# kmaninis/OSVOS-PyTorch

Measured on NVIDIA H100. Metric: frames/sec at 480x854 fwd-only, batch 1 per GPU (OSVOS.forward -> 5 logit maps), higher is better.
Workload: dtype bf16x3 (split-bf16 operands, fp32 accumulate)

## Files before the change

### include/osvos_b200.h

```cpp
#ifndef OSVOS_B200_H_
#define OSVOS_B200_H_

#include <stddef.h>
#include <stdint.h>

#ifdef __cplusplus
extern "C" {
#endif

#define OSVOS_B200_VERSION 100

#if defined(__GNUC__)
#define OSVOS_API __attribute__((visibility("default")))
#else
#define OSVOS_API
#endif

enum {
  OSVOS_OK = 0,
  OSVOS_ERR_INVALID_ARGUMENT = 1,
  OSVOS_ERR_CUDA = 2,
  OSVOS_ERR_UNSUPPORTED = 3
};

// ... 11 lines not shown
OSVOS_API int osvos_version(void);
OSVOS_API const char* osvos_last_error(void);
OSVOS_API int osvos_set_pdl(int mode);

OSVOS_API size_t osvos_packed_weight_bytes(int rows, int cols_padded);
OSVOS_API int osvos_pack_conv3x3_weights(const float* w_oihw, void* packed, int cout, int cin, int transpose_flip,
                               int col_pad, osvos_stream_t stream);

OSVOS_API int osvos_nchw_to_act(const float* x_nchw, void* act_hi, void* act_lo, int n, int c, int h, int w,
                      osvos_stream_t stream);
OSVOS_API int osvos_act_to_nchw(const void* act_hi, const void* act_lo, float* y_nchw, int n, int c, int h, int w,
                      osvos_stream_t stream);

OSVOS_API int osvos_conv_first_fwd(const float* x_nchw, const float* w_oihw, const float* bias, void* y_hi, void* y_lo,
                         int n, int h, int w, int flags, osvos_stream_t stream);

typedef struct {
  const void* x_hi;
  const void* x_lo;
  const void* w_packed;
  const float* bias;
  void* y_hi;
  void* y_lo;
  float* y_f32;
  const void* mask_hi;
  const float* proj_w;
  const float* proj_b;
  float* pq;
  void* pool_hi;
  void* pool_lo;
  float* colsum;
  int n, h, w, cin, cout;
  int flags;
} osvos_conv3x3_args;
OSVOS_API int osvos_conv3x3(const osvos_conv3x3_args* args , osvos_stream_t stream);

OSVOS_API int osvos_fold_side_weights(const float* side_w , const float* side_b ,
                                      const float* proj_w , const float* proj_b , void* packed,
                                      float* bias2 , int cin, osvos_stream_t stream);
OSVOS_API int osvos_side_folded_multi(const osvos_conv3x3_args* args , int count, osvos_stream_t stream);

typedef struct {
  const float* side_w;
  const float* side_b;
  const float* proj_w;
  const float* proj_b;
  void* packed;
  float* bias2;
  float* folded_f32;
  int cin;
} osvos_fold_item;
OSVOS_API int osvos_fold_side_weights_multi(const osvos_fold_item* items , int count, osvos_stream_t stream);
OSVOS_API int osvos_conv3x3_simt(const osvos_conv3x3_args* args , osvos_stream_t stream);

typedef struct {
  const float* x;
  const float* w1;
  const float* b1;
  const void* w2_packed;
  const float* b2;
  void* y_hi;
  void* y_lo;
  void* pool_hi;
  void* pool_lo;
  int n, h, w;
} osvos_stage1_args;
OSVOS_API int osvos_stage1_fused(const osvos_stage1_args* args , osvos_stream_t stream);

// ... 293 lines not shown
```

### osvos_pytorch_b200/_native.py

```python
import ctypes
import os
from ctypes import (POINTER, Structure, c_char_p, c_double, c_float, c_int, c_int32, c_size_t, c_uint32, c_uint64,
                    c_void_p)

_HERE = os.path.dirname(os.path.abspath(__file__))
LIB_PATH = os.path.join(_HERE, "lib", "libosvos_b200.so")

FLAG_RELU = 1
FLAG_FAST = 2
FLAG_RELU_MASK = 4
FLAG_ACCUMULATE = 8
FLAG_DEFER_FINISH = 16
FLAG_DETERMINISTIC = 32
WGRAD_FINISH_MAX = 24


class NativeLibraryError(RuntimeError):
    pass


class Conv3x3Args(Structure):
    _fields_ = [("x_hi", c_void_p), ("x_lo", c_void_p), ("w_packed", c_void_p), ("bias", c_void_p),
                ("y_hi", c_void_p), ("y_lo", c_void_p), ("y_f32", c_void_p), ("mask_hi", c_void_p),
                ("proj_w", c_void_p), ("proj_b", c_void_p), ("pq", c_void_p),
                ("pool_hi", c_void_p), ("pool_lo", c_void_p), ("colsum", c_void_p),
                ("n", c_int), ("h", c_int), ("w", c_int), ("cin", c_int), ("cout", c_int), ("flags", c_int)]


class Stage1Args(Structure):
    _fields_ = [("x", c_void_p), ("w1", c_void_p), ("b1", c_void_p), ("w2_packed", c_void_p), ("b2", c_void_p),
                ("y_hi", c_void_p), ("y_lo", c_void_p), ("pool_hi", c_void_p), ("pool_lo", c_void_p),
                ("n", c_int), ("h", c_int), ("w", c_int)]


class TailFwdArgs(Structure):
    _fields_ = [("pq", c_void_p * 4), ("fuse_bias", c_void_p), ("out", c_void_p * 5), ("label", c_void_p),
                ("sums", c_void_p), ("losses", c_void_p), ("loss_weights", c_float * 5), ("divisor", c_float),
                ("n", c_int), ("h", c_int), ("w", c_int), ("flags", c_int)]


TAIL_SUMS = 15


class TailLossBwdArgs(Structure):
    _fields_ = [("logits", c_void_p * 5), ("label", c_void_p), ("sums", c_void_p), ("upstream", c_void_p),
                ("loss_weights", c_float * 5), ("divisor", c_float), ("dpq", c_void_p * 4), ("fuse_bias_grad", c_void_p),
                ("n", c_int), ("h", c_int), ("w", c_int), ("flags", c_int)]


class WgradArgs(Structure):
    _fields_ = [("x_hi", c_void_p), ("x_lo", c_void_p), ("dz_hi", c_void_p), ("dz_lo", c_void_p), ("dw", c_void_p),
                ("workspace", c_void_p), ("n", c_int), ("h", c_int), ("w", c_int), ("cin", c_int), ("cout", c_int),
                ("dz_channels", c_int), ("flags", c_int)]


class WgradFinishItem(Structure):
    _fields_ = [("workspace", c_void_p), ("dw", c_void_p), ("cout", c_int), ("cin", c_int), ("dz_channels", c_int),
                ("accumulate", c_int), ("scale", c_float)]

# ... 43 lines not shown
                ("losses", c_void_p), ("loss_weights", c_float * 5), ("divisor", c_float), ("n", c_int), ("h", c_int),
                ("w", c_int), ("flags", c_int)]


class TailGeneralBwdArgs(Structure):
    _fields_ = [("feat", c_void_p * 4), ("pq", c_void_p * 4), ("score_w", c_void_p * 4), ("vtab", c_void_p),
                ("atab", c_void_p), ("src", c_void_p * 5), ("label", c_void_p), ("sums", c_void_p),
                ("upstream", c_void_p), ("loss_weights", c_float * 5), ("divisor", c_float), ("df_hi", c_void_p * 4),
                ("df_lo", c_void_p * 4), ("red", c_void_p * 4), ("fuse_bias_grad", c_void_p), ("workspace", c_void_p),
                ("n", c_int), ("h", c_int), ("w", c_int), ("flags", c_int)]


class UpsamplingGradsArgs(Structure):
    _fields_ = [("red", c_void_p * 4), ("upscale_w", c_void_p * 4), ("fuse_w", c_void_p), ("d_upscale_w", c_void_p * 4),
                ("d_upscale1_w", c_void_p * 4), ("d_fuse_w", c_void_p), ("d_score_w", c_void_p * 4),
                ("d_score_b", c_void_p * 4), ("d_side_b", c_void_p * 4), ("accumulate", c_int)]


UPSAMPLING_TAPS = 1360
U8_PROB, U8_BYTESCALE, U8_MASK = 0, 1, 2
RESIZE_BILINEAR, RESIZE_NEAREST = 0, 1
SGD_MAX_SEGMENTS = 64

SIGNATURES = {
    "osvos_version": (c_int, []),
    "osvos_last_error": (c_char_p, []),
    "osvos_packed_weight_bytes": (c_size_t, [c_int, c_int]),
    "osvos_pack_conv3x3_weights": (c_int, [c_void_p, c_void_p, c_int, c_int, c_int, c_int, c_void_p]),
    "osvos_nchw_to_act": (c_int, [c_void_p, c_void_p, c_void_p, c_int, c_int, c_int, c_int, c_void_p]),
    "osvos_act_to_nchw": (c_int, [c_void_p, c_void_p, c_void_p, c_int, c_int, c_int, c_int, c_void_p]),
    "osvos_conv_first_fwd": (c_int, [c_void_p, c_void_p, c_void_p, c_void_p, c_void_p, c_int, c_int, c_int, c_int,
                                     c_void_p]),
    "osvos_conv3x3": (c_int, [POINTER(Conv3x3Args), c_void_p]),
    "osvos_stage1_fused": (c_int, [POINTER(Stage1Args), c_void_p]),
    "osvos_set_pdl": (c_int, [c_int]),
    "osvos_fold_side_weights": (c_int, [c_void_p, c_void_p, c_void_p, c_void_p, c_void_p, c_void_p, c_int, c_void_p]),
    "osvos_side_folded_multi": (c_int, [POINTER(Conv3x3Args), c_int, c_void_p]),
    "osvos_fold_side_weights_multi": (c_int, [POINTER(FoldItem), c_int, c_void_p]),
    "osvos_conv3x3_simt": (c_int, [POINTER(Conv3x3Args), c_void_p]),
    "osvos_maxpool2x2_fwd": (c_int, [c_void_p, c_void_p, c_void_p, c_void_p, c_int, c_int, c_int, c_int, c_void_p]),
    "osvos_tail_fwd": (c_int, [POINTER(TailFwdArgs), c_void_p]),
    "osvos_cbce_fwd": (c_int, [c_void_p, c_void_p, c_size_t, c_double, c_void_p, c_void_p, c_void_p]),
    "osvos_cbce_bwd": (c_int, [c_void_p, c_void_p, c_void_p, c_void_p, c_double, c_size_t, c_void_p, c_void_p]),
    "osvos_wgrad_workspace_bytes": (c_size_t, [c_int, c_int]),
    "osvos_conv3x3_wgrad": (c_int, [POINTER(WgradArgs), c_void_p]),
    "osvos_wgrad_finish": (c_int, [POINTER(WgradFinishItem), c_int, c_void_p]),
    "osvos_tail_bwd": (c_int, [POINTER(TailBwdArgs), c_void_p]),
    "osvos_tail_loss_bwd": (c_int, [POINTER(TailLossBwdArgs), c_void_p]),
    "osvos_sum_f32": (c_int, [c_void_p, c_size_t, c_void_p, c_void_p, c_void_p]),
    "osvos_unpool_add_mask": (c_int, [c_void_p, c_void_p, c_void_p, c_void_p, c_void_p, c_void_p, c_void_p, c_void_p,
                                      c_int, c_int, c_int, c_int, c_void_p]),
    "osvos_side_folded_wgrad_floats": (c_size_t, [c_int]),
    "osvos_side_folded_wgrad": (c_int, [c_void_p, c_void_p, c_void_p, c_void_p, c_int, c_int, c_int, c_int, c_void_p]),
    "osvos_side_folded_wgrad_multi": (c_int, [POINTER(SideWgradItem), c_int, c_void_p]),
    "osvos_side_grads_finish": (c_int, [POINTER(SideGradsItem), c_int, c_void_p]),
    "osvos_unpool_side_mask": (c_int, [c_void_p, c_void_p, c_void_p, c_void_p, c_void_p, c_void_p, c_void_p, c_void_p,
                                       c_void_p, c_int, c_int, c_int, c_int, c_void_p]),
    "osvos_channel_sum": (c_int, [c_void_p, c_void_p, c_void_p, c_size_t, c_int, c_void_p]),
    "osvos_conv_first_bwd_workspace_bytes": (c_size_t, []),
    "osvos_conv_first_bwd": (c_int, [c_void_p, c_void_p, c_void_p, c_void_p, c_void_p, c_void_p, c_void_p, c_int, c_int, c_int,
                                     c_void_p]),
    "osvos_side_project": (c_int, [c_void_p, c_void_p, c_void_p, c_void_p, c_int, c_int, c_int, c_void_p]),
    "osvos_logits_to_u8": (c_int, [c_void_p, c_void_p, c_void_p, c_int, c_size_t, c_int, c_void_p]),
    "osvos_sgd_work_items": (c_uint32, [c_uint64, c_int, c_int]),
    "osvos_sgd_step": (c_int, [c_void_p, c_int, c_uint32, c_int, c_void_p]),
    "osvos_affine_warp": (c_int, [c_void_p, c_void_p, POINTER(c_double), POINTER(c_int), c_int, c_int, c_int, c_int,
# ... 83 lines not shown
```

### osvos_pytorch_b200/csrc/conv3x3_halo.cu

```cuda
#include "conv_common.cuh"

namespace osvos {

constexpr int kHaloRows = kTileH + 2;
constexpr int kPitch = kTileW + 2;

template <int BLOCK_N, int PLANES, bool SPLIT>
struct HaloCfg {
  static constexpr int kABoxBytes = kHaloRows * kPitch * 128;
  static constexpr int kAPlaneBytes = (kABoxBytes + 1023) / 1024 * 1024;
  static constexpr int kAStageBytes = PLANES * kAPlaneBytes;
  static constexpr int kAStages = 2;
  static constexpr int kBPlaneBytes = BLOCK_N * 128;
  static constexpr int kBStageBytes = PLANES * kBPlaneBytes;
  static constexpr int kBudget = 225 * 1024 - kAStages * kAStageBytes;
  static constexpr int kBStagesRaw = kBudget / kBStageBytes;
  static constexpr int kBStages = kBStagesRaw > 9 ? 9 : kBStagesRaw;
  static constexpr bool kSplitAcc = SPLIT;
  static_assert(!SPLIT || (PLANES == 2 && BLOCK_N <= 128), "split accumulators need two planes and 2 * BLOCK_N <= 256");
  static constexpr int kAccCols = kSplitAcc ? 2 * BLOCK_N : BLOCK_N;
  static constexpr int kAcc = kAccCols / 2;
  static constexpr int kSmemBytes = kAStages * kAStageBytes + kBStages * kBStageBytes + 1024 + 512;
  static_assert(kBStages >= 2, "weight ring too shallow");
  static_assert(kSmemBytes <= 227 * 1024, "more than the per-CTA shared memory of sm_90");
  static_assert(kSmemBytes + 4096 < (1 << 18), "descriptor start-address field would overflow");
  static_assert(kBStageBytes % 1024 == 0, "B stage must keep 1024-byte alignment");
};

template <int BLOCK_N, int PLANES, bool SPLIT, bool LEAN, bool PINGPONG, bool DET = false>
__global__ void __launch_bounds__(kConvThreads, 1)
conv3x3_halo_kernel(const __grid_constant__ CUtensorMap map_x_hi, const __grid_constant__ CUtensorMap map_x_lo,
                    const __grid_constant__ CUtensorMap map_w_hi, const __grid_constant__ CUtensorMap map_w_lo,
                    const ConvParams p) {
  using Cfg = HaloCfg<BLOCK_N, PLANES, SPLIT>;
  constexpr int SA = Cfg::kAStages, SB = Cfg::kBStages;
  constexpr int kHalves = PINGPONG ? 2 : 1;
  static_assert(!PINGPONG || kHalves * Cfg::kAcc <= 128, "a ping-pong warpgroup holds the whole tile's accumulator");

  extern __shared__ uint8_t smem_raw[];
  uint8_t* smem = reinterpret_cast<uint8_t*>((reinterpret_cast<uintptr_t>(smem_raw) + 1023) & ~uintptr_t(1023));
  uint8_t* smem_a = smem;
  uint8_t* smem_b = smem + SA * Cfg::kAStageBytes;
  uint64_t* bars = reinterpret_cast<uint64_t*>(smem_b + SB * Cfg::kBStageBytes);
  uint64_t* a_full = bars;
  uint64_t* a_empty = bars + SA;
  uint64_t* b_full = bars + 2 * SA;
  uint64_t* b_empty = bars + 2 * SA + SB;

  const int warp = threadIdx.x >> 5;
  const int lane = threadIdx.x & 31;

  if (warp == 0 && lane == 0) {
    tma_prefetch_desc(&map_x_hi);
    tma_prefetch_desc(&map_w_hi);
    if (PLANES == 2) {
      tma_prefetch_desc(&map_x_lo);
      tma_prefetch_desc(&map_w_lo);
    }
    constexpr uint32_t kReaders = PINGPONG ? 1 : 2;
    for (int i = 0; i < SA; ++i) {
      mbar_init(&a_full[i], 1);
      mbar_init(&a_empty[i], kReaders);
    }
    for (int i = 0; i < SB; ++i) {
      mbar_init(&b_full[i], 1);
      mbar_init(&b_empty[i], kReaders);
    }
    fence_barrier_init();
  }
  __syncthreads();
  pdl_wait();
  pdl_launch_dependents();

  if (warp < 4) {
    if (PINGPONG) setmaxnreg_dec<40>();
    if (warp != 0) return;
    if (elect_one()) {
      int a_stage = 0, b_stage = 0;
      uint32_t a_phase = 0, b_phase = 0;
      const bool skip_a = (p.ablate & 2) != 0, skip_b = (p.ablate & 1) != 0;
      auto issue_a = [&](int x0, int y0, int img, int kc) {
        mbar_wait(&a_empty[a_stage], a_phase ^ 1);
        if (skip_a) {
          mbar_arrive(&a_full[a_stage]);
        } else {
          uint8_t* st = smem_a + a_stage * Cfg::kAStageBytes;
          mbar_arrive_expect_tx(&a_full[a_stage], PLANES * Cfg::kABoxBytes);
          tma_load_4d(&map_x_hi, &a_full[a_stage], st, kc * kBlockK, x0, y0, img);
          if (PLANES == 2) tma_load_4d(&map_x_lo, &a_full[a_stage], st + Cfg::kAPlaneBytes, kc * kBlockK, x0, y0, img);
        }
        if (++a_stage == SA) {
          a_stage = 0;
          a_phase ^= 1;
        }
      };
      int nb = 0, tx = 0, ty = 0, img = 0;
      const int w_first = static_cast<int>(blockIdx.x), w_stride = static_cast<int>(gridDim.x);
      if (w_first < p.total_tiles) {
        decode_tile(p, w_first, nb, tx, ty, img);
        issue_a(tx * kTileW - 1, ty * kTileH - 1, img, 0);
      }
      for (int tile = w_first; tile < p.total_tiles; tile += w_stride) {
        const bool has_next = tile + w_stride < p.total_tiles;
        int nnb = 0, ntx = 0, nty = 0, nimg = 0;
        if (has_next) decode_tile(p, tile + w_stride, nnb, ntx, nty, nimg);
        const int n0 = nb * BLOCK_N;
        for (int kc = 0; kc < p.k_chunks; ++kc) {
          const int c0 = kc * kBlockK;
#pragma unroll
          for (int tap = 0; tap < 9; ++tap) {
            if (tap == 3) {
              if (kc + 1 < p.k_chunks) issue_a(tx * kTileW - 1, ty * kTileH - 1, img, kc + 1);
              else if (has_next) issue_a(ntx * kTileW - 1, nty * kTileH - 1, nimg, 0);
            }
            mbar_wait(&b_empty[b_stage], b_phase ^ 1);
            if (skip_b) {
              mbar_arrive(&b_full[b_stage]);
            } else {
              uint8_t* st = smem_b + b_stage * Cfg::kBStageBytes;
              mbar_arrive_expect_tx(&b_full[b_stage], Cfg::kBStageBytes);
              tma_load_3d(&map_w_hi, &b_full[b_stage], st, c0, n0, tap);
              if (PLANES == 2) tma_load_3d(&map_w_lo, &b_full[b_stage], st + Cfg::kBPlaneBytes, c0, n0, tap);
            }
            if (++b_stage == SB) {
              b_stage = 0;
              b_phase ^= 1;
            }
          }
        }
        nb = nnb, tx = ntx, ty = nty, img = nimg;
      }
    }
    __syncwarp();
  } else {
    if (PINGPONG) setmaxnreg_inc<232>();
    const int wg = (warp - 4) >> 2, wl = warp & 3;
    const bool leader = (threadIdx.x & 127) == 0;
    constexpr uint64_t kDescA = desc_template(16, kPitch * 128, kDescSW128);
    constexpr uint64_t kDescB = desc_template(16, 1024, kDescSW128);
    constexpr uint32_t kLoPlaneA = Cfg::kAPlaneBytes >> 4, kLoPlaneB = Cfg::kBPlaneBytes >> 4;
    constexpr uint32_t kHalfA = (8 * kPitch * 128) >> 4;
    const uint32_t smem_a_u32 = smem_u32(smem_a) + (PINGPONG ? 0 : wg * 8 * kPitch * 128), smem_b_u32 = smem_u32(smem_b);
    const bool skip_mma = (p.ablate & 4) != 0;
    float acc[kHalves][Cfg::kAcc];
    StageRelease pending;
    constexpr int kOwners = PINGPONG ? 2 : 1;
    for (int k = PINGPONG ? wg : 0;; k += kOwners) {
      const int tile = static_cast<int>(blockIdx.x) + k * static_cast<int>(gridDim.x);
      if (tile >= p.total_tiles) break;
      const bool has_next = tile + static_cast<int>(gridDim.x) < p.total_tiles;
      const int a_seq = k * p.k_chunks, b_seq = 9 * a_seq;
      int a_stage = a_seq % SA, b_stage = b_seq % SB;
      uint32_t a_phase = (a_seq / SA) & 1, b_phase = (b_seq / SB) & 1;
      if (PINGPONG && k > 0) named_bar_sync(1 + wg, 256);
#pragma unroll
      for (int h = 0; h < kHalves; ++h)
#pragma unroll
        for (int i = 0; i < Cfg::kAcc; ++i) acc[h][i] = 0.f;
      for (int kc = 0; kc < p.k_chunks; ++kc) {
        mbar_wait(&a_full[a_stage], a_phase);
        const uint64_t da0 = kDescA | static_cast<uint64_t>((smem_a_u32 + a_stage * Cfg::kAStageBytes) >> 4);
#pragma unroll
        for (int tap = 0; tap < 9; ++tap) {
          const uint32_t tap_off = static_cast<uint32_t>(((tap / 3) * kPitch + (tap % 3)) * (128 >> 4));
          mbar_wait(&b_full[b_stage], b_phase);
          if (PINGPONG && tap == 8 && kc == p.k_chunks - 1 && has_next) named_bar_arrive(1 + (wg ^ 1), 256);
          const uint64_t db_hi = kDescB | static_cast<uint64_t>((smem_b_u32 + b_stage * Cfg::kBStageBytes) >> 4);
          wgmma_fence();
#pragma unroll
          for (int h = 0; h < kHalves; ++h) {
            const uint64_t da_hi = da0 + h * kHalfA + tap_off;
            const uint64_t da_lo = da_hi + kLoPlaneA;
            if (skip_mma) continue;
#pragma unroll
            for (int ks = 0; ks < kBlockK / 16; ++ks) {
              if constexpr (Cfg::kSplitAcc) {
                wgmma_bf16<2 * BLOCK_N>(acc[h], da_hi + 2 * ks, db_hi + 2 * ks, 1);
                wgmma_bf16<BLOCK_N>(acc[h], da_lo + 2 * ks, db_hi + 2 * ks, 1);
              } else if constexpr (PLANES == 2) {
                wgmma_bf16<BLOCK_N>(acc[h], da_lo + 2 * ks, db_hi + 2 * ks, 1);
                wgmma_bf16<BLOCK_N>(acc[h], da_hi + 2 * ks, db_hi + kLoPlaneB + 2 * ks, 1);
                wgmma_bf16<BLOCK_N>(acc[h], da_hi + 2 * ks, db_hi + 2 * ks, 1);
              } else {
                wgmma_bf16<BLOCK_N>(acc[h], da_hi + 2 * ks, db_hi + 2 * ks, 1);
              }
            }
          }
          wgmma_commit();
          wgmma_wait<1>();
          pending.release(leader);
          pending.bar_b = &b_empty[b_stage];
          if (tap == 8) pending.bar_a = &a_empty[a_stage];
          if (++b_stage == SB) {
            b_stage = 0;
            b_phase ^= 1;
          }
        }
        if (++a_stage == SA) {
          a_stage = 0;
          a_phase ^= 1;
        }
      }
      wgmma_wait<0>();
#pragma unroll
      for (int h = 0; h < kHalves; ++h) wgmma_fence_operands(acc[h]);
      pending.release(leader);
#pragma unroll
      for (int h = 0; h < kHalves; ++h)
        conv_epilogue<BLOCK_N, Cfg::kSplitAcc, LEAN, DET>(p, acc[h], tile, PINGPONG ? h : wg, wl, lane);
    }
  }
}

template <int BLOCK_N, int PLANES, bool LEAN = false, bool DET = false>
static int launch_halo(const osvos_conv3x3_args* a, cudaStream_t stream) {
  constexpr bool kSplit = PLANES == 2 && BLOCK_N <= 128;
  using Cfg = HaloCfg<BLOCK_N, PLANES, kSplit>;
  ConvParams p;
  fill_conv_params(p, a, BLOCK_N);
  const int sms = device_sm_count();
  CUtensorMap mx_hi, mx_lo, mw_hi, mw_lo;
  {
    const uint64_t dims[4] = {(uint64_t)a->cin, (uint64_t)a->w, (uint64_t)a->h, (uint64_t)a->n};
    const uint64_t strides[3] = {(uint64_t)a->cin * 2, (uint64_t)a->w * a->cin * 2,
                                 (uint64_t)a->h * a->w * a->cin * 2};
    const uint32_t box[4] = {kBlockK, kPitch, kHaloRows, 1};
    int rc = encode_tensor_map(&mx_hi, CU_TENSOR_MAP_DATA_TYPE_BFLOAT16, 2, 4, a->x_hi, dims, strides, box,
                               CU_TENSOR_MAP_SWIZZLE_128B);
    if (rc) return rc;
    rc = encode_tensor_map(&mx_lo, CU_TENSOR_MAP_DATA_TYPE_BFLOAT16, 2, 4, PLANES == 2 ? a->x_lo : a->x_hi, dims,
                           strides, box, CU_TENSOR_MAP_SWIZZLE_128B);
    if (rc) return rc;
  }
  int rc = encode_weight_maps(&mw_hi, &mw_lo, a, BLOCK_N);
  if (rc) return rc;
  const int grid = p.total_tiles < sms ? p.total_tiles : sms;
  constexpr bool kCanPingPong = BLOCK_N == 64 || BLOCK_N == 128;
  const bool pingpong = kCanPingPong && p.total_tiles > 2 * sms;
  auto kern = pingpong ? conv3x3_halo_kernel<BLOCK_N, PLANES, kSplit && BLOCK_N == 64, LEAN, kCanPingPong, DET>
                       : conv3x3_halo_kernel<BLOCK_N, PLANES, kSplit, LEAN, false, DET>;
  static uint64_t attr_done[2] = {0, 0};
  OSVOS_CHECK_CUDA(ensure_dynamic_smem(kern, Cfg::kSmemBytes, &attr_done[pingpong]));
  OSVOS_CHECK_CUDA(launch_pdl(kern, dim3(grid), dim3(kConvThreads), Cfg::kSmemBytes, stream, mx_hi, mx_lo,
                              mw_hi, mw_lo, p));
  return OSVOS_OK;
}

template <bool DET>
static int conv3x3_halo_dispatch(const osvos_conv3x3_args* a, cudaStream_t stream) {
  const bool fast = (a->flags & OSVOS_FLAG_FAST) != 0;
  const bool lean = !fast && !(a->flags & OSVOS_FLAG_RELU_MASK) && a->colsum == nullptr && a->y_f32 == nullptr;
  const int m_tiles = ((a->w + kTileW - 1) / kTileW) * ((a->h + kTileH - 1) / kTileH) * a->n;
  const int sms = device_sm_count();
  const long tiles128 = static_cast<long>(m_tiles) * (a->cout / 128);
  const long waves128 = (tiles128 + sms - 1) / sms;
  const long waves256 = (static_cast<long>(m_tiles) * (a->cout / 256) + sms - 1) / sms;
  if (a->cout == 64 || (waves128 == 1 && tiles128 * 5 <= static_cast<long>(sms) * 3)) {
    if (lean) return launch_halo<64, 2, true>(a, stream);
    return fast ? launch_halo<64, 1, false, DET>(a, stream) : launch_halo<64, 2, false, DET>(a, stream);
  }
  const bool prefer256 = fast ? waves256 * 1100 < waves128 * 700 : waves256 * 2200 < waves128 * 1000;
  if (a->cout % 256 == 0 && prefer256)
    return fast ? launch_halo<256, 1, false, DET>(a, stream) : launch_halo<256, 2, false, DET>(a, stream);
  if (fast) return launch_halo<128, 1, false, DET>(a, stream);
  if (lean) return launch_halo<128, 2, true>(a, stream);
  return launch_halo<128, 2, false, DET>(a, stream);
}

static int check_conv_args(const osvos_conv3x3_args* a) {
  OSVOS_CHECK_ARG(a != nullptr);
  OSVOS_CHECK_ARG(a->n > 0 && a->h > 0 && a->w > 0);
  OSVOS_CHECK_ARG(a->cin >= 64 && a->cin % 64 == 0);
  OSVOS_CHECK_ARG(a->cout == 2 || a->cout == 16 || a->cout == 64 || (a->cout > 0 && a->cout % 128 == 0));
  OSVOS_CHECK_ARG(a->cout != 2 || (a->pq != nullptr && a->y_hi == nullptr && a->y_f32 == nullptr && a->pool_hi == nullptr &&
                                   a->colsum == nullptr && !(a->flags & (OSVOS_FLAG_RELU | OSVOS_FLAG_RELU_MASK))));
  OSVOS_CHECK_ARG(a->cout != 16 || (a->y_hi == nullptr && a->y_lo == nullptr && !(a->flags & OSVOS_FLAG_RELU_MASK)));
  OSVOS_CHECK_ARG(a->x_hi != nullptr && a->w_packed != nullptr);
  OSVOS_CHECK_ARG((a->flags & OSVOS_FLAG_FAST) || a->x_lo != nullptr);
  OSVOS_CHECK_ARG(a->y_hi != nullptr || a->y_f32 != nullptr || a->pq != nullptr || a->pool_hi != nullptr);
  OSVOS_CHECK_ARG(!(a->flags & OSVOS_FLAG_RELU_MASK) || a->mask_hi != nullptr);
  OSVOS_CHECK_ARG(a->pq == nullptr || a->cout == 2 || (a->cout == 16 && a->proj_w != nullptr));
  OSVOS_CHECK_ARG((a->pool_hi == nullptr && a->colsum == nullptr) || a->cout >= 64);
  OSVOS_CHECK_ARG((reinterpret_cast<uintptr_t>(a->x_hi) & 15) == 0);
  OSVOS_CHECK_ARG((reinterpret_cast<uintptr_t>(a->w_packed) & 15) == 0);
  OSVOS_CHECK_ARG((reinterpret_cast<uintptr_t>(a->bias) & 15) == 0);
  OSVOS_CHECK_ARG(!(a->flags & OSVOS_FLAG_DETERMINISTIC) || (reinterpret_cast<uintptr_t>(a->colsum) & 7) == 0);
  if (a->cout >= 64) {
    const uintptr_t bf16_planes = reinterpret_cast<uintptr_t>(a->y_hi) | reinterpret_cast<uintptr_t>(a->y_lo) |
                                  reinterpret_cast<uintptr_t>(a->pool_hi) | reinterpret_cast<uintptr_t>(a->pool_lo) |
                                  reinterpret_cast<uintptr_t>(a->mask_hi);
    OSVOS_CHECK_ARG((bf16_planes & 3) == 0);
    OSVOS_CHECK_ARG((reinterpret_cast<uintptr_t>(a->y_f32) & 7) == 0);
  }
// ... 2 lines not shown

}

using namespace osvos;

extern "C" int osvos_side_folded_multi(const osvos_conv3x3_args* args, int count, osvos_stream_t stream_) {
  OSVOS_CHECK_ARG(args != nullptr && count > 0 && count <= 4);
  const osvos_conv3x3_args* order[4];
  for (int k = 0; k < count; ++k) {
    int rc = check_conv_args(&args[k]);
    if (rc) return rc;
    OSVOS_CHECK_ARG(args[k].cout == 2);
    OSVOS_CHECK_ARG((args[k].flags & OSVOS_FLAG_FAST) == (args[0].flags & OSVOS_FLAG_FAST));
    order[k] = &args[k];
  }
  for (int i = 1; i < count; ++i)
    for (int j = i; j > 0 && order[j]->cin > order[j - 1]->cin; --j) {
      const osvos_conv3x3_args* t = order[j];
      order[j] = order[j - 1];
      order[j - 1] = t;
    }
  return side_conv_multi_dispatch(order, count, static_cast<cudaStream_t>(stream_));
}

extern "C" int osvos_conv3x3(const osvos_conv3x3_args* a, osvos_stream_t stream_) {
  int rc = check_conv_args(a);
  if (rc) return rc;
  cudaStream_t stream = static_cast<cudaStream_t>(stream_);
  if (a->cout == 2 || a->cout == 16) return side_conv_dispatch(a, stream);
  if ((a->flags & OSVOS_FLAG_DETERMINISTIC) && a->colsum != nullptr) return conv3x3_halo_dispatch<true>(a, stream);
  return conv3x3_halo_dispatch<false>(a, stream);
}

extern "C" size_t osvos_conv3x3_colsum_rows(int n, int h, int w) {
  if (n <= 0 || h <= 0 || w <= 0) return 0;
  return static_cast<size_t>(n) * ((h + kTileH - 1) / kTileH) * ((w + kTileW - 1) / kTileW) * 8;
}
```

### osvos_pytorch_b200/csrc/conv_common.cuh

```cuda
#pragma once
#include <stdlib.h>

#include "common.cuh"
#include "ptx.cuh"

namespace osvos {

constexpr int kTileW = 8;
constexpr int kTileH = 16;
constexpr int kBlockM = 128;
constexpr int kBlockK = 64;
constexpr int kConvThreads = 384;
constexpr int kABytes = kBlockM * kBlockK * 2;

struct ConvParams {
  const float* bias;
  __nv_bfloat16* y_hi;
  __nv_bfloat16* y_lo;
  float* y_f32;
  const __nv_bfloat16* mask_hi;
  __nv_bfloat16* pool_hi;
  __nv_bfloat16* pool_lo;
  float* colsum;
  int n, h, w, cin, cout;
  int tiles_x, tiles_y, n_blocks, total_tiles, k_chunks;
  int flags;
  int ablate;
};

__device__ __forceinline__ void decode_tile(const ConvParams& p, int tile, int& nb, int& tx, int& ty, int& img) {
  nb = tile % p.n_blocks;
  int m = tile / p.n_blocks;
  tx = m % p.tiles_x;
  m /= p.tiles_x;
  ty = m % p.tiles_y;
  img = m / p.tiles_y;
}

__device__ __forceinline__ uint32_t sw128_offset(int row, int chunk) { return row * 128 + ((chunk ^ (row & 7)) << 4); }

__device__ __forceinline__ void split_pack2(float a, float b, uint32_t& hi, uint32_t& lo) {
  asm("cvt.rn.bf16x2.f32 %0, %1, %2;" : "=r"(hi) : "f"(b), "f"(a));
  const float ra = a - __uint_as_float(hi << 16);
  const float rb = b - __uint_as_float(hi & 0xFFFF0000u);
  asm("cvt.rn.bf16x2.f32 %0, %1, %2;" : "=r"(lo) : "f"(rb), "f"(ra));
}

template <int BLOCK_N, bool SPLIT_ACC, bool LEAN = false, bool DET = false>
__device__ __forceinline__ void conv_epilogue(const ConvParams& p, const float* acc, int tile, int wg, int wl, int lane) {
  if (p.ablate & 16) return;
  int nb, tx, ty, img;
  decode_tile(p, tile, nb, tx, ty, img);
  const int lx = lane >> 2;
  const int x = tx * kTileW + lx;
  const int y0 = ty * kTileH + wg * 8 + wl * 2;
  const bool va = (y0 < p.h) && (x < p.w), vb = (y0 + 1 < p.h) && (x < p.w);
  const bool relu = (p.flags & OSVOS_FLAG_RELU) != 0;
  const bool masked = !LEAN && (p.flags & OSVOS_FLAG_RELU_MASK) != 0;
  const bool store_ok = !(p.ablate & 8);
  const size_t pix[2] = {(static_cast<size_t>(img) * p.h + y0) * p.w + x, (static_cast<size_t>(img) * p.h + y0 + 1) * p.w + x};
// ... 109 lines not shown
        st_shared_u32(act_row + h * 8 * 128 + ((j ^ lx) << 4) + col, plane ? lo : hi);
      }
    }
    fence_proxy_async_smem();
    named_bar_sync(bar_id, 128);
    if (leader && store_ok) {
      tma_store_4d(plane ? &maps.y_lo : &maps.y_hi, box, nb * 64, tx * kTileW, ty * kTileH + half * 8, img);
      bulk_commit_group();
    }
  }
}


static inline void fill_conv_params(ConvParams& p, const osvos_conv3x3_args* a, int block_n) {
  p.bias = a->bias;
  p.y_hi = static_cast<__nv_bfloat16*>(a->y_hi);
  p.y_lo = static_cast<__nv_bfloat16*>(a->y_lo);
  p.y_f32 = a->y_f32;
  p.mask_hi = static_cast<const __nv_bfloat16*>(a->mask_hi);
  p.pool_hi = static_cast<__nv_bfloat16*>(a->pool_hi);
  p.pool_lo = static_cast<__nv_bfloat16*>(a->pool_lo);
  p.colsum = a->colsum;
  p.n = a->n;
  p.h = a->h;
  p.w = a->w;
  p.cin = a->cin;
  p.cout = a->cout;
  p.tiles_x = (a->w + kTileW - 1) / kTileW;
  p.tiles_y = (a->h + kTileH - 1) / kTileH;
  p.n_blocks = a->cout / block_n;
  p.total_tiles = p.tiles_x * p.tiles_y * a->n * p.n_blocks;
  p.k_chunks = a->cin / kBlockK;
  p.flags = a->flags;
  {
    static int ablate = -1;
    if (ablate < 0) {
      const char* e = getenv("OSVOS_ABLATE");
      ablate = e ? atoi(e) : 0;
    }
    p.ablate = ablate;
  }
}

static inline int encode_weight_maps(CUtensorMap* hi, CUtensorMap* lo, const osvos_conv3x3_args* a, int block_n) {
  const size_t plane = static_cast<size_t>(9) * a->cout * a->cin;
  const uint64_t dims[3] = {(uint64_t)a->cin, (uint64_t)a->cout, 9};
  const uint64_t strides[2] = {(uint64_t)a->cin * 2, (uint64_t)a->cout * a->cin * 2};
  const uint32_t box[3] = {kBlockK, (uint32_t)block_n, 1};
  const __nv_bfloat16* wp = static_cast<const __nv_bfloat16*>(a->w_packed);
  int rc = encode_tensor_map(hi, CU_TENSOR_MAP_DATA_TYPE_BFLOAT16, 2, 3, wp, dims, strides, box,
                             CU_TENSOR_MAP_SWIZZLE_128B);
  if (rc) return rc;
  return encode_tensor_map(lo, CU_TENSOR_MAP_DATA_TYPE_BFLOAT16, 2, 3, wp + plane, dims, strides, box,
                           CU_TENSOR_MAP_SWIZZLE_128B);
}

static inline bool outputs_tma_aligned(const osvos_conv3x3_args* a) {
  return ((reinterpret_cast<uintptr_t>(a->y_hi) | reinterpret_cast<uintptr_t>(a->y_lo)) & 15) == 0;
}

static inline int encode_output_maps(OutMaps* m, const osvos_conv3x3_args* a) {
  memset(m, 0, sizeof(*m));
  const uint64_t c = a->cout;
  const uint64_t dims[4] = {c, (uint64_t)a->w, (uint64_t)a->h, (uint64_t)a->n};
  const uint64_t strides[3] = {c * 2, c * 2 * a->w, c * 2 * a->w * a->h};
  const uint32_t box[4] = {64, kTileW, kTileH / 2, 1};
// ... 15 lines not shown
```

### osvos_pytorch_b200/ops.py

```python
from ctypes import byref

import torch

from . import _native as nat


MEANVAL = (104.00699, 116.66877, 122.67892)

KERNEL_LAUNCHES = [0]


def _stream():
    return torch.cuda.current_stream().cuda_stream


def _count(n=1):
    KERNEL_LAUNCHES[0] += n


class Act:
    __slots__ = ("hi", "lo")

    def __init__(self, hi, lo):
        self.hi = hi
# ... 131 lines not shown


def side_folded(x, packed, bias2, fast=False):
    lib = nat.load()
    n, h, w, cin = x.shape
    dev = x.hi.device
    pq = torch.empty((n, h, w, 2), dtype=torch.float32, device=dev)
    a = nat.Conv3x3Args()
    a.x_hi, a.x_lo = x.hi.data_ptr(), nat.ptr(x.lo)
    a.w_packed, a.bias, a.pq = packed.data_ptr(), bias2.data_ptr(), pq.data_ptr()
    a.n, a.h, a.w, a.cin, a.cout = n, h, w, cin, 2
    a.flags = nat.FLAG_FAST if fast else 0
    _count()
    nat.check(lib.osvos_conv3x3(byref(a), _stream()), "osvos_conv3x3 (folded side branch)")
    return pq


def side_folded_multi(xs, folded, fast=False):
    lib = nat.load()
    arr = (nat.Conv3x3Args * len(xs))()
    pqs = []
    for k, (x, f) in enumerate(zip(xs, folded)):
        n, h, w, cin = x.shape
        pq = torch.empty((n, h, w, 2), dtype=torch.float32, device=x.hi.device)
        a = arr[k]
        a.x_hi, a.x_lo = x.hi.data_ptr(), nat.ptr(x.lo)
        a.w_packed, a.bias, a.pq = f[0].data_ptr(), f[1].data_ptr(), pq.data_ptr()
        a.n, a.h, a.w, a.cin, a.cout = n, h, w, cin, 2
        a.flags = nat.FLAG_FAST if fast else 0
        pqs.append(pq)
    _count()
    nat.check(lib.osvos_side_folded_multi(arr, len(xs), _stream()), "osvos_side_folded_multi")
    return pqs


def conv3x3(x, w_packed, bias, cout, relu=False, fast=False, out_act=True, out_f32=False, mask=None,
            proj_w=None, proj_b=None, simt=False, pool=False, colsum=None, deterministic=False):
    lib = nat.load()
    n, h, w, cin = x.shape
    dev = x.hi.device
    y = Act.empty(n, h, w, cout, dev, fast) if out_act else None
    yf = torch.empty((n, h, w, cout), dtype=torch.float32, device=dev) if out_f32 else None
    pq = torch.empty((n, h, w, 2), dtype=torch.float32, device=dev) if proj_w is not None else None
    a = nat.Conv3x3Args()
    a.x_hi, a.x_lo = x.hi.data_ptr(), nat.ptr(x.lo)
    a.w_packed, a.bias = w_packed.data_ptr(), nat.ptr(bias)
    a.y_hi = nat.ptr(y.hi) if y is not None else None
    a.y_lo = nat.ptr(y.lo) if y is not None else None
    a.y_f32 = nat.ptr(yf)
    a.mask_hi = nat.ptr(mask)
    a.proj_w, a.proj_b, a.pq = nat.ptr(proj_w), nat.ptr(proj_b), nat.ptr(pq)
    yp = Act.empty(n, (h + 1) // 2, (w + 1) // 2, cout, dev, fast) if pool else None
    a.pool_hi = nat.ptr(yp.hi) if pool else None
    a.pool_lo = nat.ptr(yp.lo) if pool else None
    rows = None
    if deterministic and colsum is not None:
        nrows = lib.osvos_conv3x3_colsum_rows(n, h, w)
        rows = torch.empty((nrows, cout), dtype=torch.float32, device=dev)
    a.colsum = nat.ptr(rows if rows is not None else colsum)
    a.n, a.h, a.w, a.cin, a.cout = n, h, w, cin, cout
    a.flags = (nat.FLAG_RELU if relu else 0) | (nat.FLAG_FAST if fast else 0) | \
              (nat.FLAG_RELU_MASK if mask is not None else 0) | (nat.FLAG_DETERMINISTIC if rows is not None else 0)
    fn = lib.osvos_conv3x3_simt if simt else lib.osvos_conv3x3
    _count()
    nat.check(fn(byref(a), _stream()), "osvos_conv3x3")
    if rows is not None:
        reduce_rows(rows, colsum, accumulate=True)
    if pool:
        return y, yp
    return y, yf, pq


def maxpool2x2(x):
    lib = nat.load()
    n, h, w, c = x.shape
    y = Act.empty(n, (h + 1) // 2, (w + 1) // 2, c, x.hi.device, x.lo is None)
    _count()
    nat.check(lib.osvos_maxpool2x2_fwd(x.hi.data_ptr(), nat.ptr(x.lo), y.hi.data_ptr(), nat.ptr(y.lo), n, h, w, c,
                                       _stream()), "osvos_maxpool2x2_fwd")
    return y


def side_project(feat, proj_w, proj_b):
    lib = nat.load()
    n, h, w, c = (int(v) for v in feat.shape)
    assert c == 16
    pq = torch.empty((n, h, w, 2), dtype=torch.float32, device=feat.device)
    _count()
    nat.check(lib.osvos_side_project(feat.data_ptr(), proj_w.data_ptr(), nat.ptr(proj_b), pq.data_ptr(), n, h, w,
                                     _stream()), "osvos_side_project")
    return pq


def tail_fwd(pqs, fuse_bias, n, h, w, label=None, out=None, loss_weights=None, divisor=None, deterministic=False):
    lib = nat.load()
# ... 621 lines not shown
```

Before: 652.1.

## Add stream-K scheduling for halo conv3x3 when tiles underfill the SMs

```diff
diff --git a/include/osvos_b200.h b/include/osvos_b200.h
--- a/include/osvos_b200.h
+++ b/include/osvos_b200.h
@@ -67,8 +67,12 @@
   float* colsum;
   int n, h, w, cin, cout;
   int flags;
+  float* splitk_ws;
+  unsigned* splitk_counters;
 } osvos_conv3x3_args;
 OSVOS_API int osvos_conv3x3(const osvos_conv3x3_args* args , osvos_stream_t stream);
+#define OSVOS_SPLITK_COUNTERS 4096
+OSVOS_API size_t osvos_conv3x3_splitk_workspace_bytes(const osvos_conv3x3_args* args );
 
 OSVOS_API int osvos_fold_side_weights(const float* side_w , const float* side_b ,
                                       const float* proj_w , const float* proj_b , void* packed,
diff --git a/osvos_pytorch_b200/_native.py b/osvos_pytorch_b200/_native.py
--- a/osvos_pytorch_b200/_native.py
+++ b/osvos_pytorch_b200/_native.py
@@ -13,6 +13,7 @@
 FLAG_DEFER_FINISH = 16
 FLAG_DETERMINISTIC = 32
 WGRAD_FINISH_MAX = 24
+SPLITK_COUNTERS = 4096
 
 
 class NativeLibraryError(RuntimeError):
@@ -24,7 +25,8 @@
                 ("y_hi", c_void_p), ("y_lo", c_void_p), ("y_f32", c_void_p), ("mask_hi", c_void_p),
                 ("proj_w", c_void_p), ("proj_b", c_void_p), ("pq", c_void_p),
                 ("pool_hi", c_void_p), ("pool_lo", c_void_p), ("colsum", c_void_p),
-                ("n", c_int), ("h", c_int), ("w", c_int), ("cin", c_int), ("cout", c_int), ("flags", c_int)]
+                ("n", c_int), ("h", c_int), ("w", c_int), ("cin", c_int), ("cout", c_int), ("flags", c_int),
+                ("splitk_ws", c_void_p), ("splitk_counters", c_void_p)]
 
 
 class Stage1Args(Structure):
@@ -134,6 +136,7 @@
     "osvos_conv_first_fwd": (c_int, [c_void_p, c_void_p, c_void_p, c_void_p, c_void_p, c_int, c_int, c_int, c_int,
                                      c_void_p]),
     "osvos_conv3x3": (c_int, [POINTER(Conv3x3Args), c_void_p]),
+    "osvos_conv3x3_splitk_workspace_bytes": (c_size_t, [POINTER(Conv3x3Args)]),
     "osvos_stage1_fused": (c_int, [POINTER(Stage1Args), c_void_p]),
     "osvos_set_pdl": (c_int, [c_int]),
     "osvos_fold_side_weights": (c_int, [c_void_p, c_void_p, c_void_p, c_void_p, c_void_p, c_void_p, c_int, c_void_p]),
diff --git a/osvos_pytorch_b200/csrc/conv3x3_halo.cu b/osvos_pytorch_b200/csrc/conv3x3_halo.cu
--- a/osvos_pytorch_b200/csrc/conv3x3_halo.cu
+++ b/osvos_pytorch_b200/csrc/conv3x3_halo.cu
@@ -27,7 +27,86 @@
   static_assert(kBStageBytes % 1024 == 0, "B stage must keep 1024-byte alignment");
 };
 
-template <int BLOCK_N, int PLANES, bool SPLIT, bool LEAN, bool PINGPONG, bool DET = false>
+struct Segment {
+  int tile, ub, ue;
+};
+
+__device__ __forceinline__ int sk_unit_start(const ConvParams& p, int cta) {
+  return static_cast<int>(static_cast<unsigned>(cta) * static_cast<unsigned>(p.total_tiles * 9 * p.k_chunks) / gridDim.x);
+}
+
+template <bool STREAMK>
+__device__ __forceinline__ bool first_segment(const ConvParams& p, Segment& s) {
+  const int ut = 9 * p.k_chunks;
+  if (!STREAMK) {
+    s = {static_cast<int>(blockIdx.x), 0, ut};
+    return s.tile < p.total_tiles;
+  }
+  const int u0 = sk_unit_start(p, blockIdx.x), u1 = sk_unit_start(p, blockIdx.x + 1);
+  s.tile = u0 / ut;
+  s.ub = u0 - s.tile * ut;
+  s.ue = min(u1 - s.tile * ut, ut);
+  return true;
+}
+
+template <bool STREAMK>
+__device__ __forceinline__ bool next_segment(const ConvParams& p, Segment& s) {
+  const int ut = 9 * p.k_chunks;
+  if (!STREAMK) {
+    s.tile += static_cast<int>(gridDim.x);
+    return s.tile < p.total_tiles;
+  }
+  const int u1 = sk_unit_start(p, blockIdx.x + 1), u = (s.tile + 1) * ut;
+  if (u >= u1) return false;
+  s = {s.tile + 1, 0, min(u1 - u, ut)};
+  return true;
+}
+
+template <int BLOCK_N>
+__device__ __forceinline__ bool streamk_fixup(const ConvParams& p, float* acc, int tile, volatile int* last_flag) {
+  constexpr int kPart = BLOCK_N / 2;
+  const int ut = 9 * p.k_chunks;
+  const unsigned units = static_cast<unsigned>(p.total_tiles * ut), grid = gridDim.x;
+  const int ctid = static_cast<int>(threadIdx.x) - 128;
+  const int c0 = static_cast<int>((static_cast<unsigned>(tile * ut + 1) * grid - 1) / units);
+  const int c1 = static_cast<int>((static_cast<unsigned>(tile * ut + ut) * grid - 1) / units);
+  const int me = static_cast<int>(blockIdx.x);
+  auto slot = [&](int cta) {
+    const int s = 2 * cta + (cta == c0 && sk_unit_start(p, c0) != tile * ut ? 1 : 0);
+    return reinterpret_cast<float4*>(p.sk_ws) + static_cast<size_t>(s) * (kPart / 4) * 256 + ctid;
+  };
+  float4* mine = slot(me);
+#pragma unroll
+  for (int i = 0; i < kPart / 4; ++i)
+    __stcg(mine + i * 256, make_float4(acc[4 * i], acc[4 * i + 1], acc[4 * i + 2], acc[4 * i + 3]));
+  named_bar_sync(3, 256);
+  if (ctid == 0) {
+    __threadfence();
+    const unsigned arrived = atomicAdd(p.sk_counters + tile, 1u);
+    const bool last = arrived == static_cast<unsigned>(c1 - c0);
+    if (last) {
+      p.sk_counters[tile] = 0;
+      __threadfence();
+    }
+    *last_flag = last;
+  }
+  named_bar_sync(3, 256);
+  if (!*last_flag) return false;
+  for (int c = c0; c <= c1; ++c) {
+    const float4* src = slot(c);
+#pragma unroll
+    for (int i = 0; i < kPart / 4; ++i) {
+      const float4 v = __ldcg(src + i * 256);
+      acc[4 * i] = c == c0 ? v.x : acc[4 * i] + v.x;
+      acc[4 * i + 1] = c == c0 ? v.y : acc[4 * i + 1] + v.y;
+      acc[4 * i + 2] = c == c0 ? v.z : acc[4 * i + 2] + v.z;
+      acc[4 * i + 3] = c == c0 ? v.w : acc[4 * i + 3] + v.w;
+    }
+  }
+  return true;
+}
+
+template <int BLOCK_N, int PLANES, bool SPLIT, bool LEAN, bool PINGPONG, bool DET = false, bool STREAMK = false>
 __global__ void __launch_bounds__(kConvThreads, 1)
 conv3x3_halo_kernel(const __grid_constant__ CUtensorMap map_x_hi, const __grid_constant__ CUtensorMap map_x_lo,
                     const __grid_constant__ CUtensorMap map_w_hi, const __grid_constant__ CUtensorMap map_w_lo,
@@ -36,6 +115,7 @@
   constexpr int SA = Cfg::kAStages, SB = Cfg::kBStages;
   constexpr int kHalves = PINGPONG ? 2 : 1;
   static_assert(!PINGPONG || kHalves * Cfg::kAcc <= 128, "a ping-pong warpgroup holds the whole tile's accumulator");
+  static_assert(!STREAMK || (!PINGPONG && BLOCK_N <= 128), "stream-K runs the cooperative schedule, N <= 128");
 
   extern __shared__ uint8_t smem_raw[];
   uint8_t* smem = reinterpret_cast<uint8_t*>((reinterpret_cast<uintptr_t>(smem_raw) + 1023) & ~uintptr_t(1023));
@@ -46,6 +126,7 @@
   uint64_t* a_empty = bars + SA;
   uint64_t* b_full = bars + 2 * SA;
   uint64_t* b_empty = bars + 2 * SA + SB;
+  volatile int* sk_last = reinterpret_cast<volatile int*>(bars + 2 * SA + 2 * SB);
 
   const int warp = threadIdx.x >> 5;
   const int lane = threadIdx.x & 31;
@@ -95,23 +176,28 @@
         }
       };
       int nb = 0, tx = 0, ty = 0, img = 0;
-      const int w_first = static_cast<int>(blockIdx.x), w_stride = static_cast<int>(gridDim.x);
-      if (w_first < p.total_tiles) {
-        decode_tile(p, w_first, nb, tx, ty, img);
-        issue_a(tx * kTileW - 1, ty * kTileH - 1, img, 0);
+      Segment s;
+      bool has = first_segment<STREAMK>(p, s);
+      if (has) {
+        decode_tile(p, s.tile, nb, tx, ty, img);
+        issue_a(tx * kTileW - 1, ty * kTileH - 1, img, s.ub / 9);
       }
-      for (int tile = w_first; tile < p.total_tiles; tile += w_stride) {
-        const bool has_next = tile + w_stride < p.total_tiles;
+      while (has) {
+        Segment ns = s;
+        const bool has_next = next_segment<STREAMK>(p, ns);
         int nnb = 0, ntx = 0, nty = 0, nimg = 0;
-        if (has_next) decode_tile(p, tile + w_stride, nnb, ntx, nty, nimg);
+        if (has_next) decode_tile(p, ns.tile, nnb, ntx, nty, nimg);
         const int n0 = nb * BLOCK_N;
-        for (int kc = 0; kc < p.k_chunks; ++kc) {
+        for (int kc = STREAMK ? s.ub / 9 : 0; kc < (STREAMK ? (s.ue + 8) / 9 : p.k_chunks); ++kc) {
           const int c0 = kc * kBlockK;
+          const int lo = STREAMK ? max(s.ub - 9 * kc, 0) : 0, hi = STREAMK ? min(s.ue - 9 * kc, 9) : 9;
+          const int prefetch_tap = min(max(3, lo), hi - 1);
 #pragma unroll
           for (int tap = 0; tap < 9; ++tap) {
-            if (tap == 3) {
-              if (kc + 1 < p.k_chunks) issue_a(tx * kTileW - 1, ty * kTileH - 1, img, kc + 1);
-              else if (has_next) issue_a(ntx * kTileW - 1, nty * kTileH - 1, nimg, 0);
+            if (tap < lo || tap >= hi) continue;
+            if (tap == prefetch_tap) {
+              if (9 * (kc + 1) < s.ue) issue_a(tx * kTileW - 1, ty * kTileH - 1, img, kc + 1);
+              else if (has_next) issue_a(ntx * kTileW - 1, nty * kTileH - 1, nimg, ns.ub / 9);
             }
             mbar_wait(&b_empty[b_stage], b_phase ^ 1);
             if (skip_b) {
@@ -129,6 +215,8 @@
           }
         }
         nb = nnb, tx = ntx, ty = nty, img = nimg;
+        s = ns;
+        has = has_next;
       }
     }
     __syncwarp();
@@ -144,24 +232,31 @@
     const bool skip_mma = (p.ablate & 4) != 0;
     float acc[kHalves][Cfg::kAcc];
     StageRelease pending;
-    constexpr int kOwners = PINGPONG ? 2 : 1;
-    for (int k = PINGPONG ? wg : 0;; k += kOwners) {
-      const int tile = static_cast<int>(blockIdx.x) + k * static_cast<int>(gridDim.x);
-      if (tile >= p.total_tiles) break;
+    int a_stage = 0, b_stage = 0;
+    uint32_t a_phase = 0, b_phase = 0;
+    Segment s;
+    int k = 0;
+    for (bool has = first_segment<STREAMK>(p, s); has; has = next_segment<STREAMK>(p, s), ++k) {
+      if (PINGPONG && (k & 1) != wg) continue;
+      const int tile = s.tile;
       const bool has_next = tile + static_cast<int>(gridDim.x) < p.total_tiles;
-      const int a_seq = k * p.k_chunks, b_seq = 9 * a_seq;
-      int a_stage = a_seq % SA, b_stage = b_seq % SB;
-      uint32_t a_phase = (a_seq / SA) & 1, b_phase = (b_seq / SB) & 1;
-      if (PINGPONG && k > 0) named_bar_sync(1 + wg, 256);
+      if (PINGPONG) {
+        const int a_seq = k * p.k_chunks, b_seq = 9 * a_seq;
+        a_stage = a_seq % SA, b_stage = b_seq % SB;
+        a_phase = (a_seq / SA) & 1, b_phase = (b_seq / SB) & 1;
+        if (k > 0) named_bar_sync(1 + wg, 256);
+      }
 #pragma unroll
       for (int h = 0; h < kHalves; ++h)
 #pragma unroll
         for (int i = 0; i < Cfg::kAcc; ++i) acc[h][i] = 0.f;
-      for (int kc = 0; kc < p.k_chunks; ++kc) {
+      for (int kc = STREAMK ? s.ub / 9 : 0; kc < (STREAMK ? (s.ue + 8) / 9 : p.k_chunks); ++kc) {
+        const int lo = STREAMK ? max(s.ub - 9 * kc, 0) : 0, hi = STREAMK ? min(s.ue - 9 * kc, 9) : 9;
         mbar_wait(&a_full[a_stage], a_phase);
         const uint64_t da0 = kDescA | static_cast<uint64_t>((smem_a_u32 + a_stage * Cfg::kAStageBytes) >> 4);
 #pragma unroll
         for (int tap = 0; tap < 9; ++tap) {
+          if (tap < lo || tap >= hi) continue;
           const uint32_t tap_off = static_cast<uint32_t>(((tap / 3) * kPitch + (tap % 3)) * (128 >> 4));
           mbar_wait(&b_full[b_stage], b_phase);
           if (PINGPONG && tap == 8 && kc == p.k_chunks - 1 && has_next) named_bar_arrive(1 + (wg ^ 1), 256);
@@ -190,7 +285,7 @@
           wgmma_wait<1>();
           pending.release(leader);
           pending.bar_b = &b_empty[b_stage];
-          if (tap == 8) pending.bar_a = &a_empty[a_stage];
+          if (tap == hi - 1) pending.bar_a = &a_empty[a_stage];
           if (++b_stage == SB) {
             b_stage = 0;
             b_phase ^= 1;
@@ -205,6 +300,16 @@
 #pragma unroll
       for (int h = 0; h < kHalves; ++h) wgmma_fence_operands(acc[h]);
       pending.release(leader);
+      if constexpr (STREAMK) {
+        if constexpr (Cfg::kSplitAcc) {
+#pragma unroll
+          for (int i = 0; i < Cfg::kAcc / 2; ++i) {
+            acc[0][i] += acc[0][Cfg::kAcc / 2 + i];
+            acc[0][Cfg::kAcc / 2 + i] = 0.f;
+          }
+        }
+        if ((s.ub != 0 || s.ue != 9 * p.k_chunks) && !streamk_fixup<BLOCK_N>(p, acc[0], tile, sk_last)) continue;
+      }
 #pragma unroll
       for (int h = 0; h < kHalves; ++h)
         conv_epilogue<BLOCK_N, Cfg::kSplitAcc, LEAN, DET>(p, acc[h], tile, PINGPONG ? h : wg, wl, lane);
@@ -213,7 +318,7 @@
 }
 
 template <int BLOCK_N, int PLANES, bool LEAN = false, bool DET = false>
-static int launch_halo(const osvos_conv3x3_args* a, cudaStream_t stream) {
+static int launch_halo(const osvos_conv3x3_args* a, cudaStream_t stream, int sk_grid = 0) {
   constexpr bool kSplit = PLANES == 2 && BLOCK_N <= 128;
   using Cfg = HaloCfg<BLOCK_N, PLANES, kSplit>;
   ConvParams p;
@@ -234,6 +339,18 @@
   }
   int rc = encode_weight_maps(&mw_hi, &mw_lo, a, BLOCK_N);
   if (rc) return rc;
+  if constexpr (BLOCK_N == 128) {
+    if (sk_grid > 0) {
+      p.sk_ws = a->splitk_ws;
+      p.sk_counters = a->splitk_counters;
+      auto kern = conv3x3_halo_kernel<BLOCK_N, PLANES, kSplit, LEAN, false, DET, true>;
+      static uint64_t attr_done = 0;
+      OSVOS_CHECK_CUDA(ensure_dynamic_smem(kern, Cfg::kSmemBytes, &attr_done));
+      OSVOS_CHECK_CUDA(launch_pdl(kern, dim3(sk_grid), dim3(kConvThreads), Cfg::kSmemBytes, stream, mx_hi, mx_lo,
+                                  mw_hi, mw_lo, p));
+      return OSVOS_OK;
+    }
+  }
   const int grid = p.total_tiles < sms ? p.total_tiles : sms;
   constexpr bool kCanPingPong = BLOCK_N == 64 || BLOCK_N == 128;
   const bool pingpong = kCanPingPong && p.total_tiles > 2 * sms;
@@ -246,19 +363,42 @@
   return OSVOS_OK;
 }
 
+static bool prefer_n64(const osvos_conv3x3_args* a, int sms) {
+  const long m_tiles = static_cast<long>((a->w + kTileW - 1) / kTileW) * ((a->h + kTileH - 1) / kTileH) * a->n;
+  const long tiles128 = m_tiles * (a->cout / 128);
+  return a->cout == 64 || (tiles128 <= sms && tiles128 * 5 <= static_cast<long>(sms) * 3);
+}
+
+constexpr long kFixupUnits = 12;
+static int splitk_grid(const osvos_conv3x3_args* a, int sms) {
+  if (a->cout % 128 != 0 || prefer_n64(a, sms)) return 0;
+  const long m_tiles = static_cast<long>((a->w + kTileW - 1) / kTileW) * ((a->h + kTileH - 1) / kTileH) * a->n;
+  const long tiles = m_tiles * (a->cout / 128), ut = 9L * (a->cin / kBlockK), units = tiles * ut;
+  if (tiles > 2L * sms || tiles > OSVOS_SPLITK_COUNTERS) return 0;
+  const long grid = units < sms ? units : sms;
+  if (units * grid >= (1L << 31)) return 0;
+  const long whole = (tiles + sms - 1) / sms * ut, split = (units + grid - 1) / grid + kFixupUnits;
+  return split < whole ? static_cast<int>(grid) : 0;
+}
+
 template <bool DET>
 static int conv3x3_halo_dispatch(const osvos_conv3x3_args* a, cudaStream_t stream) {
   const bool fast = (a->flags & OSVOS_FLAG_FAST) != 0;
   const bool lean = !fast && !(a->flags & OSVOS_FLAG_RELU_MASK) && a->colsum == nullptr && a->y_f32 == nullptr;
   const int m_tiles = ((a->w + kTileW - 1) / kTileW) * ((a->h + kTileH - 1) / kTileH) * a->n;
   const int sms = device_sm_count();
+  if (prefer_n64(a, sms)) {
+    if (lean) return launch_halo<64, 2, true>(a, stream);
+    return fast ? launch_halo<64, 1, false, DET>(a, stream) : launch_halo<64, 2, false, DET>(a, stream);
+  }
+  const int sk_grid = a->splitk_ws != nullptr && a->splitk_counters != nullptr ? splitk_grid(a, sms) : 0;
+  if (sk_grid > 0) {
+    if (lean) return launch_halo<128, 2, true>(a, stream, sk_grid);
+    return fast ? launch_halo<128, 1, false, DET>(a, stream, sk_grid) : launch_halo<128, 2, false, DET>(a, stream, sk_grid);
+  }
   const long tiles128 = static_cast<long>(m_tiles) * (a->cout / 128);
   const long waves128 = (tiles128 + sms - 1) / sms;
   const long waves256 = (static_cast<long>(m_tiles) * (a->cout / 256) + sms - 1) / sms;
-  if (a->cout == 64 || (waves128 == 1 && tiles128 * 5 <= static_cast<long>(sms) * 3)) {
-    if (lean) return launch_halo<64, 2, true>(a, stream);
-    return fast ? launch_halo<64, 1, false, DET>(a, stream) : launch_halo<64, 2, false, DET>(a, stream);
-  }
   const bool prefer256 = fast ? waves256 * 1100 < waves128 * 700 : waves256 * 2200 < waves128 * 1000;
   if (a->cout % 256 == 0 && prefer256)
     return fast ? launch_halo<256, 1, false, DET>(a, stream) : launch_halo<256, 2, false, DET>(a, stream);
@@ -327,6 +467,13 @@
   return conv3x3_halo_dispatch<false>(a, stream);
 }
 
+extern "C" size_t osvos_conv3x3_splitk_workspace_bytes(const osvos_conv3x3_args* a) {
+  const int sms = device_sm_count();
+  if (a == nullptr) return static_cast<size_t>(2) * sms * kBlockM * 128 * sizeof(float);
+  if (a->cout < 64 || a->n <= 0 || a->h <= 0 || a->w <= 0 || a->cin < kBlockK) return 0;
+  return static_cast<size_t>(2) * splitk_grid(a, sms) * kBlockM * 128 * sizeof(float);
+}
+
 extern "C" size_t osvos_conv3x3_colsum_rows(int n, int h, int w) {
   if (n <= 0 || h <= 0 || w <= 0) return 0;
   return static_cast<size_t>(n) * ((h + kTileH - 1) / kTileH) * ((w + kTileW - 1) / kTileW) * 8;
diff --git a/osvos_pytorch_b200/csrc/conv_common.cuh b/osvos_pytorch_b200/csrc/conv_common.cuh
--- a/osvos_pytorch_b200/csrc/conv_common.cuh
+++ b/osvos_pytorch_b200/csrc/conv_common.cuh
@@ -26,6 +26,8 @@
   int tiles_x, tiles_y, n_blocks, total_tiles, k_chunks;
   int flags;
   int ablate;
+  float* sk_ws;
+  unsigned* sk_counters;
 };
 
 __device__ __forceinline__ void decode_tile(const ConvParams& p, int tile, int& nb, int& tx, int& ty, int& img) {
@@ -201,6 +203,8 @@
   p.total_tiles = p.tiles_x * p.tiles_y * a->n * p.n_blocks;
   p.k_chunks = a->cin / kBlockK;
   p.flags = a->flags;
+  p.sk_ws = nullptr;
+  p.sk_counters = nullptr;
   {
     static int ablate = -1;
     if (ablate < 0) {
diff --git a/osvos_pytorch_b200/ops.py b/osvos_pytorch_b200/ops.py
--- a/osvos_pytorch_b200/ops.py
+++ b/osvos_pytorch_b200/ops.py
@@ -187,6 +187,22 @@
     _count()
     nat.check(lib.osvos_side_folded_multi(arr, len(xs), _stream()), "osvos_side_folded_multi")
     return pqs
+
+
+_SPLITK_WS = {}
+
+
+def _splitk_workspace(device):
+    stream = torch.cuda.current_stream(device)
+    key = (device.index, stream.cuda_stream)
+    ws = _SPLITK_WS.get(key)
+    if ws is None:
+        nbytes = nat.load().osvos_conv3x3_splitk_workspace_bytes(None)
+        with torch.cuda.device(device):
+            ws = (torch.empty(nbytes // 4, dtype=torch.float32, device=device),
+                  torch.zeros(nat.SPLITK_COUNTERS, dtype=torch.int32, device=device))
+        _SPLITK_WS[key] = ws
+    return ws
 
 
 def conv3x3(x, w_packed, bias, cout, relu=False, fast=False, out_act=True, out_f32=False, mask=None,
@@ -216,6 +232,9 @@
     a.n, a.h, a.w, a.cin, a.cout = n, h, w, cin, cout
     a.flags = (nat.FLAG_RELU if relu else 0) | (nat.FLAG_FAST if fast else 0) | \
               (nat.FLAG_RELU_MASK if mask is not None else 0) | (nat.FLAG_DETERMINISTIC if rows is not None else 0)
+    ws = _splitk_workspace(dev) if cout >= 64 and not simt else None
+    if ws is not None:
+        a.splitk_ws, a.splitk_counters = ws[0].data_ptr(), ws[1].data_ptr()
     fn = lib.osvos_conv3x3_simt if simt else lib.osvos_conv3x3
     _count()
     nat.check(fn(byref(a), _stream()), "osvos_conv3x3")
```

New measurement: 660.2, median of 6. 1.2% higher.
